# HighCWu/ControlLoRA

Hardware: AMD Instinct MI355X
Metric: train images/sec SD-1.5+ControlLoRA 512^2 bs4/GPU (higher is better)
Workload: dtype f16; 1 GPU; configs/fill50k.json on SD-1.5 topology (seeded random weights), 512x512, bs=4/GPU, fp16; hot path = hint encoder + UNet fwd/bwd + adapter AdamW; latents/text embeddings synthetic (VAE/CLIP outside the hot path); global_batch=4, parallelism=dp1, hipgraph=True, allreduce_bytes=24188160, rccl_ranks=1, comm=torch, comm_requested=auto

## Files before the change

controllora_amd/capi.py:

```python
from __future__ import annotations

import ctypes as C
import os
from typing import Optional

import torch

_HERE = os.path.dirname(os.path.abspath(__file__))
LIB_PATH = os.environ.get("CLORA_LIB_PATH") or os.path.join(_HERE, "_build", "libclora.so")

ABI_VERSION = 4
OK, ERR_ARG, ERR_LAUNCH, ERR_WORKSPACE = 0, -1, -2, -3
_ERR = {ERR_ARG: "bad argument", ERR_LAUNCH: "kernel launch failed", ERR_WORKSPACE: "workspace too small"}


class CloraError(RuntimeError):
    pass


class ConvDesc(C.Structure):
    _fields_ = [(n, C.c_int) for n in (
        "enabled", "Hin", "Win", "Cin", "Hout", "Wout", "ksize", "mul", "kmul", "off", "lim_h", "lim_w", "shift",
        "need_even", "kchunk")]

# ... 61 lines not shown

class LoraWgradJob(C.Structure):
    _fields_ = [("A", C.c_void_p), ("lda", C.c_int), ("T", C.c_void_p), ("ldt", C.c_int), ("toff", C.c_int), ("G", C.c_void_p),
                ("gs_n", C.c_int), ("gs_j", C.c_int), ("M", C.c_int), ("N", C.c_int), ("R", C.c_int), ("scale", C.c_float),
                ("a_rows", C.c_int), ("A2", C.c_void_p), ("lda2", C.c_int)]


class ConvPackJob(C.Structure):
    _fields_ = [("w", C.c_void_p), ("fwd", C.c_void_p), ("dgrad", C.c_void_p), ("Co", C.c_int), ("Ci", C.c_int), ("ksize", C.c_int),
                ("Cip", C.c_int), ("Cop", C.c_int), ("pad_", C.c_int)]


class ConvUnpackJob(C.Structure):
    _fields_ = [("stage", C.c_void_p), ("stage_b", C.c_void_p), ("grad_w", C.c_void_p), ("grad_b", C.c_void_p), ("Co", C.c_int),
                ("Ci", C.c_int), ("ksize", C.c_int), ("Cip", C.c_int)]


LORA_MAX_JOBS = 16
LORA_WGRAD_MAX_JOBS = 32
WGRAD_JOBS_PER_LAUNCH = min(LORA_WGRAD_MAX_JOBS, max(1, int(os.environ.get("CLORA_WGRAD_JOBS", "32"))))
CONV_MAX_JOBS = 32
CANNY_MAX_GROUP = 64
_P, _I, _Z, _F = C.c_void_p, C.c_int, C.c_size_t, C.c_float
_PROTOS = {
    "clora_gemm_f16": [_P, _I, _P, _P, _I, _I, _I, _I, C.POINTER(ConvDesc), C.POINTER(Epilogue), _I, _P, _Z, _P],
    "clora_gemm_f16_ex": [_P, _I, _P, _P, _I, _I, _I, _I, C.POINTER(ConvDesc), C.POINTER(Epilogue), _I, _I, _P, _Z, _P],
    "clora_conv_patch_eligible": [_I, C.POINTER(ConvDesc), _I],
    "clora_conv_strip_eligible": [_I, _I, C.POINTER(ConvDesc)],
    "clora_set_option": [C.c_char_p, _I],
    "clora_conv_wgrad_f16": [_P, _I, _P, _I, _P, _P, _I, _I, _I, C.POINTER(ConvDesc), _I, _P],
    "clora_conv_weight_pack_f32": [_P, _I, _I, _I, _I, _I, _P, _P, _P],
    "clora_conv_wgrad_unpack_f32": [_P, _P, _P, _P, _I, _I, _I, _I, _P],
    "clora_conv_weight_pack_multi_f32": [C.POINTER(ConvPackJob), _I, _P],
    "clora_conv_wgrad_unpack_multi_f32": [C.POINTER(ConvUnpackJob), _I, _P],
    "clora_attn_fwd_f16": [_P, _I, _P, _I, _P, _I, _P, _I, _P, _I, _I, _I, _I, _I, _F, _P],
    "clora_attn_max_head_dim": [_I],
    "clora_attn_fwd_causal_f16": [_P, _I, _P, _I, _P, _I, _P, _I, _I, _I, _I, _I, _F, _P],
    "clora_attn_bwd_f16": [_P, _I, _P, _I, _P, _I, _P, _I, _P, _I, _P, _P, _P, _I, _P, _I, _P, _I, _I, _I, _I, _I, _I, _F, _P, _Z, _P],
    "clora_groupnorm_fwd_f16": [_P, _P, _P, _P, _P, _I, _I, _I, _I, _F, _I, _P, _Z, _P],
    "clora_groupnorm_bwd_f16": [_P, _P, _P, _P, _P, _P, _P, _P, _P, _I, _I, _I, _I, _I, _I, _P, _Z, _P],
    "clora_groupnorm_fwd_f16_ex": [_P, _P, _I, C.POINTER(Deferred), _P, _P, _P, _P, _P, _I, _I, _I, _I, _F, _I, _P, _Z, _P],
    "clora_groupnorm_bwd_f16_ex": [_P, _P, C.POINTER(Deferred), _P, _P, _P, _I, _P, _P, _P, _P, _P, _I, _I, _I, _I, _I, _I, _P, _Z, _P],
    "clora_groupnorm_fwd_f16_team": [_P, _P, _I, C.POINTER(Deferred), _P, _P, _P, _P, _P, _I, _I, _I, _I, _F, _I, _P, _Z, _P, _Z, _P],
    "clora_groupnorm_fwd_f16_lo": [_P, _P, _I, C.POINTER(Deferred), _P, _P, _P, _P, _P, _I, _I, _I, _I, _F, _I, _P, _Z, _P, _Z, _P, _P, _P],
    "clora_layernorm_fwd_f16_lo": [_P, _P, _P, _P, _I, _I, _F, _P, _P],
    "clora_groupnorm_bwd_f16_team": [_P, _P, C.POINTER(Deferred), _P, _P, _P, _I, _P, _P, _P, _P, _P, _I, _I, _I, _I, _I, _I, _P, _Z, _P, _Z, _P],
    "clora_layernorm_bwd_f16_ex": [_P, _P, C.POINTER(Deferred), _P, _P, _P, _I, _I, _F, _P],
    "clora_finish_deferred": [C.POINTER(Deferred), _P],
    "clora_gemm_ln_fusable": [_I, _I, _I, _I, _I],
# ... 148 lines not shown
```

controllora_amd/csrc/clora_ew.hip:

```cpp
#include "clora_common.h"
#include "../../include/clora.h"

namespace {

int ew_grid(size_t work) {
    size_t b = (work + 255) / 256;
    return (int)(b > 4096 ? 4096 : (b < 1 ? 1 : b));
}

#define EW_LOOP(i, n) for (size_t i = (size_t)blockIdx.x * 256 + threadIdx.x; i < (n); i += (size_t)gridDim.x * 256)

__global__ __launch_bounds__(256) void add_kernel(const half_t* a, const half_t* b, half_t* y, size_t n8) {
    EW_LOOP(i, n8) {
        const half8 x = ld8(a + i * 8), z = ld8(b + i * 8);
        half8 o;
#pragma unroll
        for (int e = 0; e < 8; ++e) o[e] = (half_t)((float)x[e] + (float)z[e]);
        st8(y + i * 8, o);
    }
}

__global__ __launch_bounds__(256) void silu_kernel(const half_t* x, half_t* y, size_t n8) {
    EW_LOOP(i, n8) {
        const half8 v = ld8(x + i * 8);
// ... 384 lines not shown
#pragma unroll
    for (int q = 0; q < 8; ++q) s += acc[q][0] + acc[q][1] + acc[q][2] + acc[q][3];
    const unsigned long long c1 = CLORA_CYCLES(), w1 = CLORA_WALL_TICKS();
    if (threadIdx.x == 0) {
        out[3 * (size_t)blockIdx.x] = c1 - c0;
        out[3 * (size_t)blockIdx.x + 1] = w1 - w0;
        out[3 * (size_t)blockIdx.x + 2] = (unsigned long long)__float_as_uint(s);
    }
}
extern "C" int clora_clock_probe(unsigned long long* out, int blocks, int iters, void* stream) {
    if (!out || blocks <= 0 || iters <= 0) return CLORA_ERR_ARG;
    hipLaunchKernelGGL(clock_probe_kernel, dim3(blocks), dim3(256), 0, (hipStream_t)stream, out, iters);
    return clora_check_launch();
}
extern "C" int clora_abi_version(void) { return CLORA_ABI_VERSION; }
extern "C" const char* clora_build_info(void) { return "libclora gfx950 (v_mfma_f32_16x16x32_f16), ABI 2"; }

namespace {
struct ConvPackJobs { clora_conv_pack_job_t j[CLORA_CONV_MAX_JOBS]; };
struct ConvUnpackJobs { clora_conv_unpack_job_t j[CLORA_CONV_MAX_JOBS]; };

__global__ __launch_bounds__(256) void conv_weight_pack_multi_kernel(ConvPackJobs jobs) {
    const clora_conv_pack_job_t& p = jobs.j[blockIdx.y];
    const int taps = p.ksize * p.ksize, Co = p.Co, Ci = p.Ci, Cip = p.Cip, Cop = p.Cop;
    const float* w = p.w;
    half_t* fwd = (half_t*)p.fwd;
    half_t* dgrad = (half_t*)p.dgrad;
    const int nf = Co * taps * Cip, nd = dgrad ? Cip * taps * Cop : 0;
    for (int i = blockIdx.x * 256 + threadIdx.x; i < nf + nd; i += gridDim.x * 256) {
        if (i < nf) {
            const int ci = i % Cip, tap = (i / Cip) % taps, co = i / (Cip * taps);
// ... 11 lines not shown
    const int taps = p.ksize * p.ksize, Co = p.Co, Ci = p.Ci, Cip = p.Cip;
    const int nw = Co * taps * Cip;
    for (int i = blockIdx.x * 256 + threadIdx.x; i < nw + (p.grad_b ? Co : 0); i += gridDim.x * 256) {
        if (i < nw) {
            const int ci = i % Cip, tap = (i / Cip) % taps, co = i / (Cip * taps);
            const float v = p.stage[i];
            p.stage[i] = 0.f;
            if (ci < Ci) p.grad_w[((size_t)co * Ci + ci) * taps + tap] += v;
        } else {
            const int co = i - nw;
            p.grad_b[co] += p.stage_b[co];
            p.stage_b[co] = 0.f;
        }
    }
}
}

extern "C" int clora_conv_weight_pack_multi_f32(const clora_conv_pack_job_t* jobs, int njobs, void* stream) {
    if (!jobs || njobs <= 0 || njobs > CLORA_CONV_MAX_JOBS) return CLORA_ERR_ARG;
    ConvPackJobs cj;
    long most = 0;
    for (int i = 0; i < njobs; ++i) {
        const clora_conv_pack_job_t& j = jobs[i];
        if (!j.w || !j.fwd || j.Co <= 0 || j.Ci <= 0 || (j.ksize != 1 && j.ksize != 3) || j.Cip < j.Ci || (j.Cip & 7) ||
            (j.dgrad && (j.Cop < j.Co || (j.Cop & 7))))
            return CLORA_ERR_ARG;
        const int taps = j.ksize * j.ksize;
        const long total = (long)j.Co * taps * j.Cip + (j.dgrad ? (long)j.Cip * taps * j.Cop : 0);
        if (total > most) most = total;
        cj.j[i] = j;
// ... 26 lines not shown
```

controllora_amd/csrc/clora_gemm.hip:

```cpp
#include <string.h>
#include "clora_common.h"
#include "../../include/clora.h"
#include "clora_epilogue.h"

namespace {

struct GemmArgs {
    const half_t* A;
    const half_t* B;
    half_t* C;
    float* partial;
    int lda, ldc, M, N, K;
    int k_per_split;
    int tiles_n;
    int two_phase;
    int hoist_on;
    int tiles_m, n_major;
    int xg_s, xg_m, xg_n;
    clora_conv_t conv;
    clora_epilogue_t epi;
};

template <int BM, int BN, int WM, int WN>
__global__ __launch_bounds__(256) void gemm_kernel(GemmArgs p) {
// ... 1129 lines not shown
            st8(p.C + (size_t)m * p.ldc + n, finish_chunk8(p.partial, splits, p.M, p.N, p.epi, m, n));
        }
    }
}

struct WgradArgs {
    const half_t* dY;
    const half_t* X;
    float* dW;
    float* db;
    int ldy, ldx, M, N, K;
    int oihw_ci;
    int m_per_block;
    int tiles_n, tiles_k;
    clora_conv_t conv;
};

__device__ __attribute__((aligned(16))) const unsigned short g_clora_one16[8] = {0x3C00u, 0, 0, 0, 0, 0, 0, 0};

__global__ __launch_bounds__(256, 3) void conv_wgrad_kernel(WgradArgs p) {
    constexpr int BMR = 64, NST = 3;
    constexpr int SUB = BMR * 16;
    constexpr int STAGE = 8 * SUB;
    __shared__ __attribute__((aligned(16))) half_t smem[NST * STAGE];
    const int t = threadIdx.x;
    const int tile = blockIdx.x;
    const int tn = tile % p.tiles_n, tk = tile / p.tiles_n;
    const int n0 = tn * 64, k0 = tk * 64;
    const int mbeg = blockIdx.y * p.m_per_block;
    const int mend = (mbeg + p.m_per_block < p.M) ? mbeg + p.m_per_block : p.M;
    const int nst = (mend - mbeg + BMR - 1) / BMR;
    const bool conv = p.conv.enabled != 0;
    const half_t* zero_page = reinterpret_cast<const half_t*>(g_clora_zero16);
    const half_t* one_page = reinterpret_cast<const half_t*>(g_clora_one16);

    const int w = t >> 6, l = t & 63, g = l >> 4, li = l & 15;
    const int lm = (w & 1) * 32 + (l >> 1);
    const int c8 = (l & 1) * 8;
    int ncol[2], kcol[2], ky[2], kx[2], ci[2];
    bool n_ok[2], k_ok[2], k_one[2];
#pragma unroll
    for (int q = 0; q < 2; ++q) {
        const int sub = q * 2 + (w >> 1);
        ncol[q] = n0 + sub * 16 + c8;
        kcol[q] = k0 + sub * 16 + c8;
        n_ok[q] = ncol[q] < p.N;
        k_ok[q] = kcol[q] < p.K;
        k_one[q] = p.db != nullptr && kcol[q] == p.K;
        ky[q] = 0; kx[q] = 0; ci[q] = kcol[q];
        if (conv && k_ok[q]) {
            const int tap = kcol[q] / p.conv.Cin;
            ci[q] = kcol[q] - tap * p.conv.Cin;
            ky[q] = tap / p.conv.ksize;
            kx[q] = tap - ky[q] * p.conv.ksize;
        }
    }
    int mrow = mbeg + lm;
    auto issue_stage = [&](int buf) {
        half_t* base = smem + buf * STAGE + (w & 1) * 512;
        const bool mok = mrow < mend;
        size_t xrow = 0;
        int ty0 = 0, tx0 = 0;
        if (mok) {
// ... 71 lines not shown
#pragma unroll
            for (int i = 0; i < 2; ++i)
#pragma unroll
                for (int j = 0; j < 2; ++j) acc[i][j] = mfma16(af[i], bf[j], acc[i][j]);
        }
    }
    CLORA_WAIT_VMCNT(0);
#pragma unroll
    for (int i = 0; i < 2; ++i)
#pragma unroll
        for (int j = 0; j < 2; ++j)
#pragma unroll
            for (int r = 0; r < 4; ++r) {
                const int n = n0 + wm * 32 + i * 16 + 4 * g + r;
                const int kk = k0 + wn * 32 + j * 16 + li;
                if (n < p.N && kk < p.K) {
                    if (p.oihw_ci > 0) {
                        const int cin = p.conv.enabled ? p.conv.Cin : p.K;
                        const int tap = kk / cin, ci = kk - tap * cin;
                        const int taps = p.conv.enabled ? p.conv.ksize * p.conv.ksize : 1;
                        if (ci < p.oihw_ci) atomicAdd(p.dW + ((size_t)n * p.oihw_ci + ci) * taps + tap, acc[i][j][r]);
                    } else {
                        atomicAdd(p.dW + (size_t)n * p.K + kk, acc[i][j][r]);
                    }
                } else if (n < p.N && kk == p.K && p.db) atomicAdd(p.db + n, acc[i][j][r]);
            }
}

struct WgradPatchArgs {
    const half_t* dY;
    const half_t* X;
    float* dW;
    float* db;
    int N, K, H, W, nimg, nseg, rows_per_block, row_chunks;
    int Hin, Win;
};

template <int CIN, int NFW, int TW, int STRIDE = 1>
__global__ __launch_bounds__(CIN / 16 * 128) void conv_wgrad_patch_kernel(WgradPatchArgs p) {
    constexpr int WC = CIN / 16, NW = WC * 2, NP = 2 * NFW;
    constexpr int PW = STRIDE == 1 ? TW + 2 : 2 * TW + 1, PPIX = 3 * PW;
    constexpr int P_NI = (PPIX * 2 + 63) / 64;
    constexpr int PLANE = P_NI * 512;
    constexpr int Y_NI = TW * 2 / 64, YPLANE = TW * 16;
    constexpr int BUF = WC * PLANE + NP * YPLANE;
    constexpr int NI = WC * P_NI + NP * Y_NI, NIW = (NI + NW - 1) / NW;
    constexpr int KS = TW / 32;
    static_assert((2 * BUF + 512) * 2 <= 160 * 1024, "LDS per workgroup");
    __shared__ __attribute__((aligned(16))) half_t smem[2 * BUF + 512];
    const int t = threadIdx.x, w = t >> 6, l = t & 63, g = l >> 4, li = l & 15;
    const int cb = w >> 1, wn = w & 1;
    const half_t* zero_page = reinterpret_cast<const half_t*>(g_clora_zero16);

// ... 88 lines not shown
                const half_t* q = P + (ky * PW + koff + s * 32) * 16 + troff;
                const half4v lo = CLORA_DS_READ_TR16(q), hi = CLORA_DS_READ_TR16(q + 64);
                const half8 bf = half8{lo[0], lo[1], lo[2], lo[3], hi[0], hi[1], hi[2], hi[3]};
#pragma unroll
                for (int f = 0; f < NFW; ++f) acc[tap][f] = mfma16(af[f], bf, acc[tap][f]);
            }
        }
        CLORA_RAW_BARRIER();
    }
    CLORA_WAIT_VMCNT(0);
#pragma unroll
    for (int f = 0; f < NFW; ++f)
#pragma unroll
        for (int r = 0; r < 4; ++r) {
            const int n = (wn * NFW + f) * 16 + 4 * g + r;
            if (n < p.N) {
#pragma unroll
                for (int tap = 0; tap < 9; ++tap) atomicAdd(p.dW + (size_t)n * p.K + tap * CIN + cb * 16 + li, acc[tap][f][r]);
                if (cb == 0 && li == 0 && p.db) atomicAdd(p.db + n, accb[f][r]);
            }
        }
}

template <int CIN, int NFW, int TW, int STRIDE = 1>
int launch_wgrad_patch(WgradPatchArgs& a, hipStream_t s) {
    a.nseg = a.W / TW;
    const long strips = (long)a.nimg * a.nseg;
    long target = 4700000L / ((long)a.N * (a.K + 1));
    target = target < 64 ? 64 : (target > 512 ? 512 : target);
    if (clora_option(CLORA_OPT_WGRAD_PATCH) >= 64) target = clora_option(CLORA_OPT_WGRAD_PATCH);
    long rpb = ((long)a.H * strips + target - 1) / target;
    if (rpb < 4) rpb = 4;
    if (rpb > a.H) rpb = a.H;
    a.rows_per_block = (int)rpb;
    a.row_chunks = clora_cdiv(a.H, rpb);
    hipLaunchKernelGGL((conv_wgrad_patch_kernel<CIN, NFW, TW, STRIDE>), dim3((unsigned)(strips * a.row_chunks)), dim3(CIN / 16 * 128), 0, s, a);
    return clora_check_launch();
}

struct StripArgs {
    const half_t* X;
    const half_t* Wt;
    half_t* C;
    const float* bias;
    int N, ldc, H, W, nimg, nseg, rows_per_block, row_chunks;
    int off, kmul;
};

template <int CIN, int NF, int TW>
__global__ __launch_bounds__(256) void conv3x3_strip_kernel(StripArgs p) {
    constexpr int WC = CIN / 16, NW = 4, KSTEPS = CIN / 32;
// ... 774 lines not shown
}

extern "C" int clora_conv_weight_pack_f32(const float* w, int Co, int Ci, int ksize, int Cip, int Cop, clora_half* fwd,
                                          clora_half* dgrad, void* stream) {
    if (!w || !fwd || Co <= 0 || Ci <= 0 || (ksize != 1 && ksize != 3) || Cip < Ci || (Cip & 7) || (dgrad && (Cop < Co || (Cop & 7))))
        return CLORA_ERR_ARG;
    const int taps = ksize * ksize;
    const long total = (long)Co * taps * Cip + (dgrad ? (long)Cip * taps * Cop : 0);
    int blocks = (int)((total + 255) / 256);
    if (blocks > 2048) blocks = 2048;
    hipLaunchKernelGGL(conv_weight_pack_kernel, dim3(blocks), dim3(256), 0, (hipStream_t)stream, w, Co, Ci, taps, Cip, Cop,
                       (half_t*)fwd, (half_t*)dgrad);
    return clora_check_launch();
}

extern "C" int clora_conv_wgrad_f16(const clora_half* dY, int ldy, const clora_half* X, int ldx, float* dW, float* db,
                                    int M, int N, int K, const clora_conv_t* conv, int oihw_ci, void* stream) {
    if (!dY || !X || !dW || M <= 0 || N <= 0 || K <= 0 || (K & 7) || (N & 7) || (ldy & 7) || oihw_ci < 0) return CLORA_ERR_ARG;
    WgradArgs a;
    a.dY = (const half_t*)dY; a.X = (const half_t*)X; a.dW = dW; a.db = db;
    a.ldy = ldy; a.ldx = ldx; a.M = M; a.N = N; a.K = K; a.oihw_ci = oihw_ci;
    if (conv && conv->enabled) {
        a.conv = *conv;
        if ((conv->Cin & 7) || K != conv->ksize * conv->ksize * conv->Cin || conv->kchunk != 0) return CLORA_ERR_ARG;
    } else {
        a.conv = clora_conv_t();
        a.conv.enabled = 0;
        if (ldx & 7) return CLORA_ERR_ARG;
    }
    if (conv && conv->enabled && clora_option(CLORA_OPT_WGRAD_PATCH) && oihw_ci == 0 && ldy == N) {
        const clora_conv_t& c = *conv;
        const bool s1 = c.ksize == 3 && c.mul == 1 && c.kmul == 1 && c.off == -1 && c.shift == 0 && c.need_even == 0 && c.Hout == c.Hin &&
                        c.Wout == c.Win && c.lim_h == c.Hin && c.lim_w == c.Win && c.Hout > 0 && (M % (c.Hout * c.Wout)) == 0 &&
                        (long)M * (c.Cin > N ? c.Cin : N) < (1L << 31);
        const bool s2 = c.ksize == 3 && c.mul == 2 && c.kmul == 1 && c.off == 0 && c.shift == 0 && c.need_even == 0 && c.Hin == 2 * c.Hout &&
                        c.Win == 2 * c.Wout && c.lim_h == c.Hin && c.lim_w == c.Win && c.Hout > 0 && (M % (c.Hout * c.Wout)) == 0 &&
                        (long)M * 4 * (c.Cin > N ? c.Cin : N) < (1L << 31);
        if ((s1 || s2) && (c.Cin == 32 || c.Cin == 64) && N <= 64) {
            WgradPatchArgs q;
            q.dY = (const half_t*)dY; q.X = (const half_t*)X; q.dW = dW; q.db = db; q.N = N; q.K = K; q.H = c.Hout; q.W = c.Wout;
            q.Hin = c.Hin; q.Win = c.Win;
            q.nimg = M / (c.Hout * c.Wout);
            hipStream_t s = (hipStream_t)stream;
            if (s2) {
                if (c.Cin == 32 && N <= 32 && (c.Wout % 64) == 0) return launch_wgrad_patch<32, 1, 64, 2>(q, s);
                if (c.Cin == 32 && N <= 64 && (c.Wout % 64) == 0) return launch_wgrad_patch<32, 2, 64, 2>(q, s);
                if (c.Cin == 64 && N <= 64 && (c.Wout % 64) == 0) return launch_wgrad_patch<64, 2, 64, 2>(q, s);
            } else {
            if (c.Cin == 32 && N <= 32 && (c.Wout % 128) == 0) return launch_wgrad_patch<32, 1, 128>(q, s);
            if (c.Cin == 32 && N <= 64 && (c.Wout % 128) == 0) return launch_wgrad_patch<32, 2, 128>(q, s);
            if (c.Cin == 32 && N <= 64 && (c.Wout % 64) == 0) return launch_wgrad_patch<32, 2, 64>(q, s);
            if (c.Cin == 64 && N <= 64 && (c.Wout % 64) == 0) return launch_wgrad_patch<64, 2, 64>(q, s);
            }
        }
    }
    a.tiles_n = clora_cdiv(N, 64);
    a.tiles_k = clora_cdiv(K + (db ? 8 : 0), 64);
    const int tiles = a.tiles_n * a.tiles_k;
    int chunks = clora_cdiv(2048, tiles);
    int mpb = clora_cdiv(clora_cdiv(M, chunks), 64) * 64;
    if (mpb < 256) mpb = 256;
    a.m_per_block = mpb;
    hipLaunchKernelGGL(conv_wgrad_kernel, dim3(tiles, clora_cdiv(M, mpb)), dim3(256), 0, (hipStream_t)stream, a);
    return clora_check_launch();
}
```

controllora_amd/kernels.py:

```python
from __future__ import annotations

import ctypes as C
import os
from typing import Optional, Tuple

import torch

from . import capi
from .capi import ConvDesc, Epilogue, ptr

f16, f32 = torch.float16, torch.float32


class KernelProfiler:

    def __init__(self, detail=False):
        self.detail = detail
        self.records = []

    def summary(self):
        torch.cuda.synchronize()
        agg = {}
        for name, e0, e1, fl, by in self.records:
            a = agg.setdefault(name, dict(calls=0, ms=0.0, flops=0.0, bytes=0.0))
# ... 328 lines not shown

def conv_wgrad_staged(dY, X, M, N, K, conv, stage: torch.Tensor, weight_grad: torch.Tensor, bias_grad: Optional[torch.Tensor], Cip: int):
    assert stage.dtype == f32 and stage.numel() == N * K + N and weight_grad.dtype == f32 and weight_grad.is_contiguous()
    sw, sb = stage[:N * K], stage[N * K:]
    _call("clora_conv_wgrad_f16", ptr(dY, f16), N, ptr(X, f16), K, ptr(sw), ptr(sb), M, N, K,
          C.byref(conv) if conv is not None else None, 0, flops=2.0 * M * N * K)
    if bias_grad is not None and conv_unpack_defer(conv_unpack_job(stage, weight_grad, bias_grad, Cip), stage, weight_grad, bias_grad):
        return
    Co, Ci, k, _ = weight_grad.shape
    _call("clora_conv_wgrad_unpack_f32", ptr(sw), ptr(sb) if bias_grad is not None else None, ptr(weight_grad),
          ptr(bias_grad, f32) if bias_grad is not None else None, Co, Ci, k, Cip)
    if bias_grad is None:
        sb.zero_()


def conv_weight_pack(weight: torch.Tensor, Cip: int, need_dgrad: bool, out=None):
    Co, Ci, k, _ = weight.shape
    Cop = (Co + 7) // 8 * 8
    if out is not None:
        fwd, dgrad = out
    else:
        fwd = torch.empty((Co, k * k * Cip), dtype=f16, device=weight.device)
        dgrad = torch.empty((Cip, k * k * Cop), dtype=f16, device=weight.device) if need_dgrad else None
    _call("clora_conv_weight_pack_f32", ptr(weight, f32), Co, Ci, k, Cip, Cop, ptr(fwd), ptr(dgrad) if dgrad is not None else None)
    return fwd, dgrad


def conv_pack_job(weight: torch.Tensor, Cip: int, fwd: torch.Tensor, dgrad: Optional[torch.Tensor]):
    Co, Ci, k, _ = weight.shape
    assert weight.dtype == f32 and weight.is_contiguous() and fwd.dtype == f16 and fwd.numel() == Co * k * k * Cip
# ... 301 lines not shown


def lora_wgrad_multi(jobs, device):
    groups = {}
    for j in jobs:
        groups.setdefault(4 if j.R <= 4 else (8 if j.R <= 8 else 16), []).append(j)
    wsb = capi.lib().cdll.clora_lora_wgrad_workspace_bytes
    for _, js in groups.items():
        for i in range(0, len(js), capi.WGRAD_JOBS_PER_LAUNCH):
            chunk = js[i:i + capi.WGRAD_JOBS_PER_LAUNCH]
            ws = workspace(sum(wsb(j.M, j.N, j.R) for j in chunk), device)
            arr = (capi.LoraWgradJob * len(chunk))(*chunk)
            _call("clora_lora_wgrad_multi_f16", arr, len(chunk), ptr(ws), ws.numel(), nbytes=sum(2.0 * j.M * j.N for j in chunk))


_wgrad_queue = {"jobs": [], "refs": [], "task": None, "enabled": os.environ.get("CLORA_DEFER_WGRAD", "1") != "0", "unpack": []}
DEFER_UNPACK = os.environ.get("CLORA_DEFER_UNPACK", "1") != "0"


def _graph_task_id():
    f = getattr(torch._C, "_current_graph_task_id", None)
    return f() if f is not None else -1


def _defer_open():
    if not _wgrad_queue["enabled"] or PROFILER is not None:
        return False
    task = _graph_task_id()
    if task < 0:
        return False
    if _wgrad_queue["task"] != task:
# ... 8 lines not shown
        lora_wgrad_multi(jobs, device)
        return
    _wgrad_queue["jobs"].extend(jobs)
    _wgrad_queue["refs"].extend(keepalive)
    _wgrad_queue["device"] = device


def conv_unpack_defer(job, *keepalive) -> bool:
    if not DEFER_UNPACK or not _defer_open():
        return False
    _wgrad_queue["unpack"].append(job)
    _wgrad_queue["refs"].extend(keepalive)
    return True


def lora_wgrad_discard():
    _wgrad_queue["jobs"].clear()
    _wgrad_queue["unpack"].clear()
    _wgrad_queue["refs"].clear()
    _wgrad_queue["task"] = None


def lora_wgrad_flush():
    jobs, _wgrad_queue["jobs"] = _wgrad_queue["jobs"], []
    unpack, _wgrad_queue["unpack"] = _wgrad_queue["unpack"], []
    _wgrad_queue["task"] = None
    if unpack:
        conv_wgrad_unpack_multi(unpack)
    if jobs:
        batches = []
        for j in jobs:
            for b in batches:
                if len(b[0]) < capi.WGRAD_JOBS_PER_LAUNCH and j.G not in b[1] and b[2] == (4 if j.R <= 4 else (8 if j.R <= 8 else 16)):
                    b[0].append(j); b[1].add(j.G)
                    break
            else:
                batches.append(([j], {j.G}, 4 if j.R <= 4 else (8 if j.R <= 8 else 16)))
        for b in batches:
            lora_wgrad_multi(b[0], _wgrad_queue["device"])
    _wgrad_queue["refs"].clear()


def lora_up(base, T, toff, U, M, N, scale, out=None, u_tr=False):
# ... 187 lines not shown
```

controllora_amd/ops.py:

```python
from __future__ import annotations

from typing import List, Optional, Sequence, Tuple

import torch

from . import kernels as K

f16, f32 = torch.float16, torch.float32


class LinearPack:

    def __init__(self, weight: torch.Tensor, bias: Optional[torch.Tensor], pad_n_to: int = 8):
        w = weight.detach().reshape(weight.shape[0], -1).to(f16)
        N, Kd = w.shape
        if Kd % 8:
            w = torch.cat([w, w.new_zeros(N, 8 - Kd % 8)], 1)
            Kd = w.shape[1]
        Np = (N + pad_n_to - 1) // pad_n_to * pad_n_to
        if Np != N:
            w = torch.cat([w, w.new_zeros(Np - N, Kd)], 0)
        self.N, self.K, self.N_logical = Np, Kd, N
        self.w = w.contiguous()
        self.wt = w.t().contiguous()
# ... 1305 lines not shown
                K.lora_wgrad(a_, t_, 0, g_, gn, gj, M, n_, R, scale=sc_)
        dbase, dx = dy, None
        if ctx.same:
            if ctx.needs_input_grad[0] or ctx.needs_input_grad[1]:
                dbase = K.lora_up(dy, dT, 0, D.detach(), M, D.shape[1], 1.0, u_tr=True)
            return dbase, None, None, None, None
        if ctx.needs_input_grad[1]:
            dx = K.lora_up(None, dT, 0, D.detach(), M, D.shape[1], 1.0, u_tr=True)
        return dbase, dx, None, None, None


def lora_apply(base, x, down_weight, up_weight, scale):
    return _LoraApplyFn.apply(base, x, down_weight, up_weight, float(scale))


class _TrainConvFn(torch.autograd.Function):

    @staticmethod
    def forward(ctx, x, weight, bias, B, H, W, stride, asym_pad, need_dx):
        Co, Ci, k, _ = weight.shape
        Cip = x.shape[1]
        if PERSISTENT_CONV_PACKS:
            wp, wd = TRAIN_CONV_PACKS.get(weight, Cip, need_dx)
        else:
            wp, wd = K.conv_weight_pack(weight.detach(), Cip, need_dx)
        if k == 3:
            cd, Ho, Wo = K.conv_fwd_desc(H, W, Cip, 3, stride, 0 if asym_pad else 1, False, asym_pad)
            y = K.gemm(x, wp, B * Ho * Wo, Co, 9 * Cip, conv=cd, bias=bias.detach())
        else:
            cd, Ho, Wo = None, H, W
# ... 10 lines not shown
        weight, bias = ctx.params
        B, H, W, Ho, Wo, stride, asym_pad, need_dx, cd = ctx.cfg
        Co, Ci, k, _ = weight.shape
        Cip = x.shape[1]
        Cop = (Co + 7) // 8 * 8
        M = B * Ho * Wo
        dx = None
        if need_dx:
            if k == 3:
                cdd = K.conv_dgrad_desc(Ho, Wo, Cop, H, W, 3, stride, 1, asym_pad)
                dx = K.gemm(dy, ctx.wd, B * H * W, Cip, 9 * Cop, conv=cdd)
            else:
                dx = K.gemm(dy, ctx.wd, M, Cip, Cop)
        if weight.requires_grad:
            gb = _grad_buffer(bias) if bias.requires_grad else None
            if k == 1:
                K.conv_wgrad_into(dy, x, M, Co, Cip, cd, _grad_buffer(weight), gb)
            else:
                stage = getattr(weight, "_clora_wgrad_stage", None)
                if stage is None or stage.numel() != Co * 9 * Cip + Co or stage.device != dy.device:
                    stage = torch.zeros(Co * 9 * Cip + Co, dtype=f32, device=dy.device)
                    weight._clora_wgrad_stage = stage
                K.conv_wgrad_staged(dy, x, M, Co, 9 * Cip, cd, stage, _grad_buffer(weight), gb, Cip)
        return dx, None, None, None, None, None, None, None, None


def train_conv(x, weight, bias, B, H, W, stride=1, asym_pad=False, need_dx=True):
    return _TrainConvFn.apply(x, weight, bias, B, H, W, stride, asym_pad, need_dx)
```

include/clora.h:

```cpp
#ifndef CLORA_H
#define CLORA_H
#include <stddef.h>
#include <stdint.h>

#ifdef __cplusplus
extern "C" {
#endif

#define CLORA_OK 0
#define CLORA_ERR_ARG (-1)
#define CLORA_ERR_LAUNCH (-2)
#define CLORA_ERR_WORKSPACE (-3)

typedef uint16_t clora_half;

typedef struct {
    int enabled;
    int Hin, Win, Cin;
    int Hout, Wout;
    int ksize;
    int mul, kmul, off, lim_h, lim_w, shift, need_even;
    int kchunk;
} clora_conv_t;

// ... 97 lines not shown
    const float* w;
    clora_half* fwd;
    clora_half* dgrad;
    int Co, Ci, ksize, Cip, Cop, pad_;
} clora_conv_pack_job_t;
int clora_conv_weight_pack_multi_f32(const clora_conv_pack_job_t* jobs, int njobs, void* stream);
typedef struct {
    float* stage;
    float* stage_b;
    float* grad_w;
    float* grad_b;
    int Co, Ci, ksize, Cip;
} clora_conv_unpack_job_t;
int clora_conv_wgrad_unpack_multi_f32(const clora_conv_unpack_job_t* jobs, int njobs, void* stream);

int clora_attn_fwd_f16(const clora_half* q, int ldq, const clora_half* k, int ldk, const clora_half* v, int ldv,
                       clora_half* o, int ldo, float* lse, int B, int H, int Nq, int Nk, int D, float scale,
                       void* stream);
int clora_attn_max_head_dim(int backward);
int clora_attn_fwd_causal_f16(const clora_half* q, int ldq, const clora_half* k, int ldk, const clora_half* v, int ldv,
                              clora_half* o, int ldo, int B, int H, int N, int D, float scale, void* stream);
int clora_attn_bwd_f16(const clora_half* q, int ldq, const clora_half* k, int ldk, const clora_half* v, int ldv,
                       const clora_half* o, int ldo, const clora_half* dO, int lddo, const float* lse,
                       float* delta, clora_half* dq, int lddq, clora_half* dk, int lddk, clora_half* dv, int lddv,
                       int B, int H, int Nq, int Nk, int D, float scale, void* workspace, size_t workspace_bytes,
                       void* stream);

int clora_groupnorm_fwd_f16(const clora_half* x, clora_half* y, const float* gamma, const float* beta, float* stats,
                            int B, int HW, int C, int G, float eps, int fuse_silu, void* workspace,
                            size_t workspace_bytes, void* stream);
// ... 154 lines not shown
```

Before: 184.2 images/s.

## Replace atomic conv weight-grad accumulation with per-chunk slabs and deferred fold

Conv weight-gradient kernels now write partial sums into per-row-chunk fp32 slabs in a workspace instead of atomically adding into the gradient, or staging then unpacking. A new multi-job fold kernel reduces the slabs, converts them to OIHW layout and accumulates into grad_w/grad_b, and it can be deferred and batched with the other wgrad flush work. The aim is to remove atomic contention and the separate stage/unpack pass. In exchange it adds workspace memory and an extra read of every slab. It is enabled by default through CLORA_WGRAD_SLABS.

```diff
diff --git a/controllora_amd/capi.py b/controllora_amd/capi.py
--- a/controllora_amd/capi.py
+++ b/controllora_amd/capi.py
@@ -99,6 +99,17 @@
 class ConvUnpackJob(C.Structure):
     _fields_ = [("stage", C.c_void_p), ("stage_b", C.c_void_p), ("grad_w", C.c_void_p), ("grad_b", C.c_void_p), ("Co", C.c_int),
                 ("Ci", C.c_int), ("ksize", C.c_int), ("Cip", C.c_int)]
+
+
+class WgradPlan(C.Structure):
+    _fields_ = [("kernel", C.c_int), ("blocks", C.c_int), ("row_chunks", C.c_int), ("rows_per_chunk", C.c_int), ("nslabs", C.c_int),
+                ("kw", C.c_int), ("slab_stride", C.c_int), ("patch_cin", C.c_int), ("patch_nfw", C.c_int), ("patch_tw", C.c_int),
+                ("patch_stride", C.c_int), ("workspace_bytes", C.c_size_t)]
+
+
+class ConvFoldJob(C.Structure):
+    _fields_ = [("slabs", C.c_void_p), ("grad_w", C.c_void_p), ("grad_b", C.c_void_p), ("nslabs", C.c_int), ("kw", C.c_int),
+                ("slab_stride", C.c_int), ("Co", C.c_int), ("Ci", C.c_int), ("ksize", C.c_int), ("Cip", C.c_int)]
 
 
 LORA_MAX_JOBS = 16
@@ -118,6 +129,9 @@
     "clora_conv_wgrad_unpack_f32": [_P, _P, _P, _P, _I, _I, _I, _I, _P],
     "clora_conv_weight_pack_multi_f32": [C.POINTER(ConvPackJob), _I, _P],
     "clora_conv_wgrad_unpack_multi_f32": [C.POINTER(ConvUnpackJob), _I, _P],
+    "clora_conv_wgrad_slab_plan": [_I, _I, _I, C.POINTER(ConvDesc), _I, _I, C.POINTER(WgradPlan)],
+    "clora_conv_wgrad_slabs_f16": [_P, _P, _I, _I, _I, C.POINTER(ConvDesc), _I, _I, _P, _Z, _P],
+    "clora_conv_wgrad_fold_multi_f32": [C.POINTER(ConvFoldJob), _I, _P],
     "clora_attn_fwd_f16": [_P, _I, _P, _I, _P, _I, _P, _I, _P, _I, _I, _I, _I, _I, _F, _P],
     "clora_attn_max_head_dim": [_I],
     "clora_attn_fwd_causal_f16": [_P, _I, _P, _I, _P, _I, _P, _I, _I, _I, _I, _I, _F, _P],
diff --git a/controllora_amd/csrc/clora_ew.hip b/controllora_amd/csrc/clora_ew.hip
--- a/controllora_amd/csrc/clora_ew.hip
+++ b/controllora_amd/csrc/clora_ew.hip
@@ -422,7 +422,9 @@
     return clora_check_launch();
 }
 extern "C" int clora_abi_version(void) { return CLORA_ABI_VERSION; }
-extern "C" const char* clora_build_info(void) { return "libclora gfx950 (v_mfma_f32_16x16x32_f16), ABI 2"; }
+#define CLORA_STR_(x) #x
+#define CLORA_STR(x) CLORA_STR_(x)
+extern "C" const char* clora_build_info(void) { return "libclora gfx950 (v_mfma_f32_16x16x32_f16), ABI " CLORA_STR(CLORA_ABI_VERSION); }
 
 namespace {
 struct ConvPackJobs { clora_conv_pack_job_t j[CLORA_CONV_MAX_JOBS]; };
@@ -464,6 +466,80 @@
         }
     }
 }
+struct ConvFoldJobs { clora_conv_fold_job_t j[CLORA_CONV_MAX_JOBS]; int lanes[CLORA_CONV_MAX_JOBS]; };
+
+__global__ __launch_bounds__(256) void conv_wgrad_fold_multi_kernel(ConvFoldJobs jobs) {
+    __shared__ floatx4 red[256];
+    const clora_conv_fold_job_t& p = jobs.j[blockIdx.y];
+    const int L = jobs.lanes[blockIdx.y], EPB = 256 / L;
+    const int t = threadIdx.x, e = t % EPB, q = t / EPB;
+    const int taps = p.ksize * p.ksize, kq = taps * p.Cip / 4;
+    const int nq = p.Co * kq, total = nq + (p.grad_b ? p.Co : 0);
+    const size_t stride = (size_t)p.slab_stride;
+    for (int base = blockIdx.x * EPB; base < total; base += gridDim.x * EPB) {
+        const int i = base + e;
+        int co = 0, col = 0;
+        floatx4 s = zero4f();
+        if (i < nq) {
+            co = i / kq; col = (i - co * kq) * 4;
+            const float* src = p.slabs + (size_t)co * p.kw + col;
+            for (int b = q; b < p.nslabs; b += 8 * L) {
+                floatx4 v[8];
+#pragma unroll
+                for (int u = 0; u < 8; ++u)
+                    v[u] = (b + u * L < p.nslabs) ? *reinterpret_cast<const floatx4*>(src + (size_t)(b + u * L) * stride) : zero4f();
+#pragma unroll
+                for (int u = 0; u < 8; ++u) s += v[u];
+            }
+        } else if (i < total) {
+            co = i - nq;
+            const float* src = p.slabs + (size_t)co * p.kw + kq * 4;
+            for (int b = q; b < p.nslabs; b += L) s[0] += src[(size_t)b * stride];
+        }
+        red[t] = s;
+        __syncthreads();
+        if (q == 0 && i < total) {
+            for (int u = 1; u < L; ++u) {
+                s += red[u * EPB + e];
+            }
+            if (i < nq) {
+                const int tap = col / p.Cip, ci = col - tap * p.Cip;
+                float* dst = p.grad_w + ((size_t)co * p.Ci + ci) * taps + tap;
+                if (ci < p.Ci) dst[0] += s[0];
+                if (ci + 1 < p.Ci) dst[taps] += s[1];
+                if (ci + 2 < p.Ci) dst[2 * taps] += s[2];
+                if (ci + 3 < p.Ci) dst[3 * taps] += s[3];
+            } else {
+                p.grad_b[co] += s[0];
+            }
+        }
+        __syncthreads();
+    }
+}
+}
+
+extern "C" int clora_conv_wgrad_fold_multi_f32(const clora_conv_fold_job_t* jobs, int njobs, void* stream) {
+    if (!jobs || njobs <= 0 || njobs > CLORA_CONV_MAX_JOBS) return CLORA_ERR_ARG;
+    ConvFoldJobs cj;
+    int most = 0;
+    for (int i = 0; i < njobs; ++i) {
+        const clora_conv_fold_job_t& j = jobs[i];
+        if (!j.slabs || !j.grad_w || j.Co <= 0 || j.Ci <= 0 || j.Cip < j.Ci || (j.ksize != 1 && j.ksize != 3) || j.nslabs <= 0) return CLORA_ERR_ARG;
+        const long kcols = (long)j.ksize * j.ksize * j.Cip;
+        if (j.kw != kcols + (j.grad_b ? 8 : 0) || (long)j.slab_stride != (long)j.Co * j.kw) return CLORA_ERR_ARG;
+        for (int k = 0; k < i; ++k)
+            if (jobs[k].grad_w == j.grad_w) return CLORA_ERR_ARG;
+        if ((j.Cip & 3) || ((size_t)j.slabs & 15)) return CLORA_ERR_ARG;
+        int L = 1;
+        while (L < 32 && j.nslabs > 8 * L) L *= 2;
+        const int groups = clora_cdiv((long)j.Co * kcols / 4 + (j.grad_b ? j.Co : 0), 256 / L);
+        if (groups > most) most = groups;
+        cj.j[i] = j;
+        cj.lanes[i] = L;
+    }
+    if (most > 2048) most = 2048;
+    hipLaunchKernelGGL(conv_wgrad_fold_multi_kernel, dim3(most, njobs), dim3(256), 0, (hipStream_t)stream, cj);
+    return clora_check_launch();
 }
 
 extern "C" int clora_conv_weight_pack_multi_f32(const clora_conv_pack_job_t* jobs, int njobs, void* stream) {
diff --git a/controllora_amd/csrc/clora_gemm.hip b/controllora_amd/csrc/clora_gemm.hip
--- a/controllora_amd/csrc/clora_gemm.hip
+++ b/controllora_amd/csrc/clora_gemm.hip
@@ -1167,10 +1167,13 @@
     int m_per_block;
     int tiles_n, tiles_k;
     clora_conv_t conv;
+    int has_bias;
+    int kw, slab_stride;
 };
 
 __device__ __attribute__((aligned(16))) const unsigned short g_clora_one16[8] = {0x3C00u, 0, 0, 0, 0, 0, 0, 0};
 
+template <bool SLAB>
 __global__ __launch_bounds__(256, 3) void conv_wgrad_kernel(WgradArgs p) {
     constexpr int BMR = 64, NST = 3;
     constexpr int SUB = BMR * 16;
@@ -1199,7 +1202,7 @@
         kcol[q] = k0 + sub * 16 + c8;
         n_ok[q] = ncol[q] < p.N;
         k_ok[q] = kcol[q] < p.K;
-        k_one[q] = p.db != nullptr && kcol[q] == p.K;
+        k_one[q] = p.has_bias && kcol[q] == p.K;
         ky[q] = 0; kx[q] = 0; ci[q] = kcol[q];
         if (conv && k_ok[q]) {
             const int tap = kcol[q] / p.conv.Cin;
@@ -1301,7 +1304,10 @@
             for (int r = 0; r < 4; ++r) {
                 const int n = n0 + wm * 32 + i * 16 + 4 * g + r;
                 const int kk = k0 + wn * 32 + j * 16 + li;
-                if (n < p.N && kk < p.K) {
+                if constexpr (SLAB) {
+                    if (n < p.N && (kk < p.K || (kk == p.K && p.has_bias)))
+                        p.dW[(size_t)blockIdx.y * p.slab_stride + (size_t)n * p.kw + kk] = acc[i][j][r];
+                } else if (n < p.N && kk < p.K) {
                     if (p.oihw_ci > 0) {
                         const int cin = p.conv.enabled ? p.conv.Cin : p.K;
                         const int tap = kk / cin, ci = kk - tap * cin;
@@ -1321,9 +1327,10 @@
     float* db;
     int N, K, H, W, nimg, nseg, rows_per_block, row_chunks;
     int Hin, Win;
+    int has_bias, kw, slab_stride;
 };
 
-template <int CIN, int NFW, int TW, int STRIDE = 1>
+template <int CIN, int NFW, int TW, int STRIDE = 1, bool SLAB = false>
 __global__ __launch_bounds__(CIN / 16 * 128) void conv_wgrad_patch_kernel(WgradPatchArgs p) {
     constexpr int WC = CIN / 16, NW = WC * 2, NP = 2 * NFW;
     constexpr int PW = STRIDE == 1 ? TW + 2 : 2 * TW + 1, PPIX = 3 * PW;
@@ -1442,7 +1449,14 @@
 #pragma unroll
         for (int r = 0; r < 4; ++r) {
             const int n = (wn * NFW + f) * 16 + 4 * g + r;
-            if (n < p.N) {
+            if constexpr (SLAB) {
+                if (n < p.N) {
+                    float* row = p.dW + (size_t)blockIdx.x * p.slab_stride + (size_t)n * p.kw;
+#pragma unroll
+                    for (int tap = 0; tap < 9; ++tap) row[tap * CIN + cb * 16 + li] = acc[tap][f][r];
+                    if (cb == 0 && li == 0 && p.has_bias) row[p.K] = accb[f][r];
+                }
+            } else if (n < p.N) {
 #pragma unroll
                 for (int tap = 0; tap < 9; ++tap) atomicAdd(p.dW + (size_t)n * p.K + tap * CIN + cb * 16 + li, acc[tap][f][r]);
                 if (cb == 0 && li == 0 && p.db) atomicAdd(p.db + n, accb[f][r]);
@@ -1450,19 +1464,28 @@
         }
 }
 
-template <int CIN, int NFW, int TW, int STRIDE = 1>
+constexpr int WGRAD_SLAB_PATCH_BLOCKS = 512;
+constexpr int WGRAD_SLAB_GATHER_BLOCKS = 2048, WGRAD_SLAB_GATHER_MIN_ROWS = 512, WGRAD_SLAB_GATHER_MAX_CHUNKS = 256;
+static void wgrad_patch_blocks(int N, int K, int H, long strips, bool slab, int chunks, int* rows_per_block, int* row_chunks) {
+    long target = slab ? WGRAD_SLAB_PATCH_BLOCKS : 4700000L / ((long)N * (K + 1));
+    if (!slab) target = target < 64 ? 64 : (target > 512 ? 512 : target);
+    const bool forced = clora_option(CLORA_OPT_WGRAD_PATCH) >= 64;
+    if (forced) target = clora_option(CLORA_OPT_WGRAD_PATCH);
+    long rpb = ((long)H * strips + target - 1) / target;
+    const long least = (slab && !forced) ? 8 : 4;
+    if (rpb < least) rpb = least;
+    if (slab && chunks > 0) rpb = clora_cdiv(H, chunks);
+    if (rpb > H) rpb = H;
+    *rows_per_block = (int)rpb;
+    *row_chunks = clora_cdiv(H, (int)rpb);
+}
+
+template <int CIN, int NFW, int TW, int STRIDE = 1, bool SLAB = false>
 int launch_wgrad_patch(WgradPatchArgs& a, hipStream_t s) {
     a.nseg = a.W / TW;
     const long strips = (long)a.nimg * a.nseg;
-    long target = 4700000L / ((long)a.N * (a.K + 1));
-    target = target < 64 ? 64 : (target > 512 ? 512 : target);
-    if (clora_option(CLORA_OPT_WGRAD_PATCH) >= 64) target = clora_option(CLORA_OPT_WGRAD_PATCH);
-    long rpb = ((long)a.H * strips + target - 1) / target;
-    if (rpb < 4) rpb = 4;
-    if (rpb > a.H) rpb = a.H;
-    a.rows_per_block = (int)rpb;
-    a.row_chunks = clora_cdiv(a.H, rpb);
-    hipLaunchKernelGGL((conv_wgrad_patch_kernel<CIN, NFW, TW, STRIDE>), dim3((unsigned)(strips * a.row_chunks)), dim3(CIN / 16 * 128), 0, s, a);
+    if (!SLAB) wgrad_patch_blocks(a.N, a.K, a.H, strips, false, 0, &a.rows_per_block, &a.row_chunks);
+    hipLaunchKernelGGL((conv_wgrad_patch_kernel<CIN, NFW, TW, STRIDE, SLAB>), dim3((unsigned)(strips * a.row_chunks)), dim3(CIN / 16 * 128), 0, s, a);
     return clora_check_launch();
 }
 
@@ -2267,6 +2290,42 @@
     return clora_check_launch();
 }
 
+struct WgradPatchPick { int cin, nfw, tw, stride; };
+static bool wgrad_patch_pick(int M, int N, const clora_conv_t* conv, bool wide, WgradPatchPick* k) {
+    if (!conv || !conv->enabled || !clora_option(CLORA_OPT_WGRAD_PATCH)) return false;
+    const clora_conv_t& c = *conv;
+    const bool s1 = c.ksize == 3 && c.mul == 1 && c.kmul == 1 && c.off == -1 && c.shift == 0 && c.need_even == 0 && c.Hout == c.Hin &&
+                    c.Wout == c.Win && c.lim_h == c.Hin && c.lim_w == c.Win && c.Hout > 0 && (M % (c.Hout * c.Wout)) == 0 &&
+                    (long)M * (c.Cin > N ? c.Cin : N) < (1L << 31);
+    const bool s2 = c.ksize == 3 && c.mul == 2 && c.kmul == 1 && c.off == 0 && c.shift == 0 && c.need_even == 0 && c.Hin == 2 * c.Hout &&
+                    c.Win == 2 * c.Wout && c.lim_h == c.Hin && c.lim_w == c.Win && c.Hout > 0 && (M % (c.Hout * c.Wout)) == 0 &&
+                    (long)M * 4 * (c.Cin > N ? c.Cin : N) < (1L << 31);
+    if (!(s1 || s2) || (c.Cin != 32 && c.Cin != 64)) return false;
+    const int nfw = N <= 32 ? 1 : (N <= 64 ? 2 : 4);
+    if (s2) {
+        if (N > 64 || (c.Wout % 64)) return false;
+        *k = WgradPatchPick{c.Cin, c.Cin == 64 ? 2 : nfw, 64, 2};
+        return true;
+    }
+    if (c.Cin == 32 && N <= 64 && (c.Wout % 128) == 0) { *k = WgradPatchPick{32, nfw, 128, 1}; return true; }
+    if (c.Cin == 32 && N <= 64 && (c.Wout % 64) == 0) { *k = WgradPatchPick{32, 2, 64, 1}; return true; }
+    if (c.Cin == 64 && N <= 64 && (c.Wout % 64) == 0) { *k = WgradPatchPick{64, 2, 64, 1}; return true; }
+    if (wide && c.Cin == 64 && N <= 128 && (c.Wout % 64) == 0) { *k = WgradPatchPick{64, 4, 64, 1}; return true; }
+    return false;
+}
+
+template <bool SLAB>
+static int launch_wgrad_patch_pick(const WgradPatchPick& k, WgradPatchArgs& q, hipStream_t s) {
+#define CLORA_WGRAD_PATCH_CASE(CIN, NFW, TW, ST) \
+    if (k.cin == CIN && k.nfw == NFW && k.tw == TW && k.stride == ST) return launch_wgrad_patch<CIN, NFW, TW, ST, SLAB>(q, s);
+    CLORA_WGRAD_PATCH_CASE(32, 1, 64, 2) CLORA_WGRAD_PATCH_CASE(32, 2, 64, 2) CLORA_WGRAD_PATCH_CASE(64, 2, 64, 2)
+    CLORA_WGRAD_PATCH_CASE(32, 1, 128, 1) CLORA_WGRAD_PATCH_CASE(32, 2, 128, 1) CLORA_WGRAD_PATCH_CASE(32, 2, 64, 1)
+    CLORA_WGRAD_PATCH_CASE(64, 2, 64, 1)
+    if constexpr (SLAB) { CLORA_WGRAD_PATCH_CASE(64, 4, 64, 1) }
+#undef CLORA_WGRAD_PATCH_CASE
+    return CLORA_ERR_ARG;
+}
+
 extern "C" int clora_conv_wgrad_f16(const clora_half* dY, int ldy, const clora_half* X, int ldx, float* dW, float* db,
                                     int M, int N, int K, const clora_conv_t* conv, int oihw_ci, void* stream) {
     if (!dY || !X || !dW || M <= 0 || N <= 0 || K <= 0 || (K & 7) || (N & 7) || (ldy & 7) || oihw_ci < 0) return CLORA_ERR_ARG;
@@ -2281,31 +2340,16 @@
         a.conv.enabled = 0;
         if (ldx & 7) return CLORA_ERR_ARG;
     }
-    if (conv && conv->enabled && clora_option(CLORA_OPT_WGRAD_PATCH) && oihw_ci == 0 && ldy == N) {
+    a.has_bias = db != nullptr; a.kw = 0; a.slab_stride = 0;
+    WgradPatchPick pick;
+    if (oihw_ci == 0 && ldy == N && wgrad_patch_pick(M, N, conv, false, &pick)) {
         const clora_conv_t& c = *conv;
-        const bool s1 = c.ksize == 3 && c.mul == 1 && c.kmul == 1 && c.off == -1 && c.shift == 0 && c.need_even == 0 && c.Hout == c.Hin &&
-                        c.Wout == c.Win && c.lim_h == c.Hin && c.lim_w == c.Win && c.Hout > 0 && (M % (c.Hout * c.Wout)) == 0 &&
-                        (long)M * (c.Cin > N ? c.Cin : N) < (1L << 31);
-        const bool s2 = c.ksize == 3 && c.mul == 2 && c.kmul == 1 && c.off == 0 && c.shift == 0 && c.need_even == 0 && c.Hin == 2 * c.Hout &&
-                        c.Win == 2 * c.Wout && c.lim_h == c.Hin && c.lim_w == c.Win && c.Hout > 0 && (M % (c.Hout * c.Wout)) == 0 &&
-                        (long)M * 4 * (c.Cin > N ? c.Cin : N) < (1L << 31);
-        if ((s1 || s2) && (c.Cin == 32 || c.Cin == 64) && N <= 64) {
-            WgradPatchArgs q;
-            q.dY = (const half_t*)dY; q.X = (const half_t*)X; q.dW = dW; q.db = db; q.N = N; q.K = K; q.H = c.Hout; q.W = c.Wout;
-            q.Hin = c.Hin; q.Win = c.Win;
-            q.nimg = M / (c.Hout * c.Wout);
-            hipStream_t s = (hipStream_t)stream;
-            if (s2) {
-                if (c.Cin == 32 && N <= 32 && (c.Wout % 64) == 0) return launch_wgrad_patch<32, 1, 64, 2>(q, s);
-                if (c.Cin == 32 && N <= 64 && (c.Wout % 64) == 0) return launch_wgrad_patch<32, 2, 64, 2>(q, s);
-                if (c.Cin == 64 && N <= 64 && (c.Wout % 64) == 0) return launch_wgrad_patch<64, 2, 64, 2>(q, s);
-            } else {
-            if (c.Cin == 32 && N <= 32 && (c.Wout % 128) == 0) return launch_wgrad_patch<32, 1, 128>(q, s);
-            if (c.Cin == 32 && N <= 64 && (c.Wout % 128) == 0) return launch_wgrad_patch<32, 2, 128>(q, s);
-            if (c.Cin == 32 && N <= 64 && (c.Wout % 64) == 0) return launch_wgrad_patch<32, 2, 64>(q, s);
-            if (c.Cin == 64 && N <= 64 && (c.Wout % 64) == 0) return launch_wgrad_patch<64, 2, 64>(q, s);
-            }
-        }
+        WgradPatchArgs q;
+        q.dY = (const half_t*)dY; q.X = (const half_t*)X; q.dW = dW; q.db = db; q.N = N; q.K = K; q.H = c.Hout; q.W = c.Wout;
+        q.Hin = c.Hin; q.Win = c.Win;
+        q.nimg = M / (c.Hout * c.Wout);
+        q.has_bias = db != nullptr; q.kw = 0; q.slab_stride = 0;
+        return launch_wgrad_patch_pick<false>(pick, q, (hipStream_t)stream);
     }
     a.tiles_n = clora_cdiv(N, 64);
     a.tiles_k = clora_cdiv(K + (db ? 8 : 0), 64);
@@ -2314,6 +2358,72 @@
     int mpb = clora_cdiv(clora_cdiv(M, chunks), 64) * 64;
     if (mpb < 256) mpb = 256;
     a.m_per_block = mpb;
-    hipLaunchKernelGGL(conv_wgrad_kernel, dim3(tiles, clora_cdiv(M, mpb)), dim3(256), 0, (hipStream_t)stream, a);
+    hipLaunchKernelGGL(conv_wgrad_kernel<false>, dim3(tiles, clora_cdiv(M, mpb)), dim3(256), 0, (hipStream_t)stream, a);
     return clora_check_launch();
 }
+
+static int wgrad_conv_args_ok(int M, int N, int K, const clora_conv_t* conv) {
+    if (M <= 0 || N <= 0 || K <= 0 || (K & 7) || (N & 7)) return 0;
+    if (conv && conv->enabled && ((conv->Cin & 7) || K != conv->ksize * conv->ksize * conv->Cin || conv->kchunk != 0)) return 0;
+    return 1;
+}
+
+extern "C" int clora_conv_wgrad_slab_plan(int M, int N, int K, const clora_conv_t* conv, int with_bias, int chunks, clora_wgrad_plan_t* plan) {
+    if (!plan || chunks < 0 || !wgrad_conv_args_ok(M, N, K, conv)) return CLORA_ERR_ARG;
+    clora_wgrad_plan_t& p = *plan;
+    p = clora_wgrad_plan_t();
+    p.kw = K + (with_bias ? 8 : 0);
+    if ((long)N * p.kw >= (1L << 31)) return CLORA_ERR_ARG;
+    p.slab_stride = N * p.kw;
+    WgradPatchPick pick;
+    if (wgrad_patch_pick(M, N, conv, true, &pick)) {
+        const long strips = (long)(M / (conv->Hout * conv->Wout)) * (conv->Wout / pick.tw);
+        p.kernel = 1;
+        p.patch_cin = pick.cin; p.patch_nfw = pick.nfw; p.patch_tw = pick.tw; p.patch_stride = pick.stride;
+        wgrad_patch_blocks(N, K, conv->Hout, strips, true, chunks, &p.rows_per_chunk, &p.row_chunks);
+        p.blocks = (int)(strips * p.row_chunks);
+        p.nslabs = p.blocks;
+    } else {
+        const int tiles = clora_cdiv(N, 64) * clora_cdiv(p.kw, 64);
+        int want = chunks > 0 ? chunks : clora_cdiv(WGRAD_SLAB_GATHER_BLOCKS, tiles);
+        if (chunks == 0 && want > WGRAD_SLAB_GATHER_MAX_CHUNKS) want = WGRAD_SLAB_GATHER_MAX_CHUNKS;
+        int mpb = clora_cdiv(clora_cdiv(M, want), 64) * 64;
+        if (mpb < WGRAD_SLAB_GATHER_MIN_ROWS && chunks == 0) mpb = WGRAD_SLAB_GATHER_MIN_ROWS;
+        p.kernel = 0;
+        p.rows_per_chunk = mpb;
+        p.row_chunks = clora_cdiv(M, mpb);
+        p.blocks = tiles * p.row_chunks;
+        p.nslabs = p.row_chunks;
+    }
+    p.workspace_bytes = (size_t)p.nslabs * p.slab_stride * sizeof(float);
+    return CLORA_OK;
+}
+
+extern "C" int clora_conv_wgrad_slabs_f16(const clora_half* dY, const clora_half* X, int M, int N, int K, const clora_conv_t* conv,
+                                          int with_bias, int chunks, float* workspace, size_t workspace_bytes, void* stream) {
+    clora_wgrad_plan_t p;
+    if (!dY || !X || !workspace) return CLORA_ERR_ARG;
+    if (int rc = clora_conv_wgrad_slab_plan(M, N, K, conv, with_bias, chunks, &p)) return rc;
+    if (workspace_bytes < p.workspace_bytes) return CLORA_ERR_WORKSPACE;
+    if (p.kernel == 1) {
+        const clora_conv_t& c = *conv;
+        WgradPatchArgs q;
+        q.dY = (const half_t*)dY; q.X = (const half_t*)X; q.dW = workspace; q.db = nullptr; q.N = N; q.K = K; q.H = c.Hout; q.W = c.Wout;
+        q.Hin = c.Hin; q.Win = c.Win;
+        q.nimg = M / (c.Hout * c.Wout);
+        q.has_bias = with_bias != 0; q.kw = p.kw; q.slab_stride = p.slab_stride;
+        q.rows_per_block = p.rows_per_chunk; q.row_chunks = p.row_chunks;
+        return launch_wgrad_patch_pick<true>(WgradPatchPick{p.patch_cin, p.patch_nfw, p.patch_tw, p.patch_stride}, q, (hipStream_t)stream);
+    }
+    WgradArgs a;
+    a.dY = (const half_t*)dY; a.X = (const half_t*)X; a.dW = workspace; a.db = nullptr;
+    a.ldy = N; a.ldx = K; a.M = M; a.N = N; a.K = K; a.oihw_ci = 0;
+    if (conv && conv->enabled) a.conv = *conv;
+    else { a.conv = clora_conv_t(); a.conv.enabled = 0; }
+    a.has_bias = with_bias != 0; a.kw = p.kw; a.slab_stride = p.slab_stride;
+    a.tiles_n = clora_cdiv(N, 64);
+    a.tiles_k = clora_cdiv(p.kw, 64);
+    a.m_per_block = p.rows_per_chunk;
+    hipLaunchKernelGGL(conv_wgrad_kernel<true>, dim3(a.tiles_n * a.tiles_k, p.row_chunks), dim3(256), 0, (hipStream_t)stream, a);
+    return clora_check_launch();
+}
diff --git a/controllora_amd/kernels.py b/controllora_amd/kernels.py
--- a/controllora_amd/kernels.py
+++ b/controllora_amd/kernels.py
@@ -366,6 +366,50 @@
         sb.zero_()
 
 
+WGRAD_SLABS = os.environ.get("CLORA_WGRAD_SLABS", "1") != "0"
+
+
+def conv_wgrad_plan(M: int, N: int, K: int, conv: Optional[ConvDesc], with_bias: bool, chunks: int = 0) -> capi.WgradPlan:
+    plan = capi.WgradPlan()
+    capi.lib().call("clora_conv_wgrad_slab_plan", M, N, K, C.byref(conv) if conv is not None else None, int(with_bias), int(chunks),
+                    C.byref(plan))
+    return plan
+
+
+def conv_fold_job(ws: torch.Tensor, plan: capi.WgradPlan, weight_grad: torch.Tensor, bias_grad: Optional[torch.Tensor], Cip: int):
+    Co, Ci, k, _ = weight_grad.shape
+    assert weight_grad.dtype == f32 and weight_grad.is_contiguous() and ws.dtype == f32 and ws.numel() * 4 >= plan.workspace_bytes
+    assert plan.kw == k * k * Cip + (8 if bias_grad is not None else 0) and plan.slab_stride == Co * plan.kw
+    return capi.ConvFoldJob(ptr(ws), ptr(weight_grad), ptr(bias_grad, f32) if bias_grad is not None else None, plan.nslabs, plan.kw,
+                            plan.slab_stride, Co, Ci, k, Cip)
+
+
+def conv_wgrad_fold_multi(jobs):
+    for i in range(0, len(jobs), capi.CONV_MAX_JOBS):
+        chunk = jobs[i:i + capi.CONV_MAX_JOBS]
+        arr = (capi.ConvFoldJob * len(chunk))(*chunk)
+        _call("clora_conv_wgrad_fold_multi_f32", arr, len(chunk), nbytes=sum(4.0 * j.nslabs * j.slab_stride for j in chunk))
+
+
+def conv_wgrad_slabs_launch(dY, X, M, N, K, conv, with_bias: bool, ws: torch.Tensor, chunks: int = 0):
+    assert ws.dtype == f32 and dY.dtype == f16 and X.dtype == f16 and dY.is_contiguous() and X.is_contiguous()
+    _call("clora_conv_wgrad_slabs_f16", ptr(dY, f16), ptr(X, f16), M, N, K, C.byref(conv) if conv is not None else None,
+          int(with_bias), int(chunks), ptr(ws), ws.numel() * 4, flops=2.0 * M * N * K)
+
+
+def conv_wgrad_slabs(dY, X, M, N, K, conv, ws: torch.Tensor, weight_grad: torch.Tensor, bias_grad: Optional[torch.Tensor], Cip: int,
+                     chunks: int = 0):
+    plan = conv_wgrad_plan(M, N, K, conv, bias_grad is not None, chunks)
+    job = conv_fold_job(ws, plan, weight_grad, bias_grad, Cip)
+    deferred = conv_fold_open(job)
+    conv_wgrad_slabs_launch(dY, X, M, N, K, conv, bias_grad is not None, ws, chunks)
+    if deferred:
+        conv_fold_defer(job, ws, weight_grad, bias_grad)
+    else:
+        conv_wgrad_fold_multi([job])
+    return plan
+
+
 def conv_weight_pack(weight: torch.Tensor, Cip: int, need_dgrad: bool, out=None):
     Co, Ci, k, _ = weight.shape
     Cop = (Co + 7) // 8 * 8
@@ -697,7 +741,7 @@
             _call("clora_lora_wgrad_multi_f16", arr, len(chunk), ptr(ws), ws.numel(), nbytes=sum(2.0 * j.M * j.N for j in chunk))
 
 
-_wgrad_queue = {"jobs": [], "refs": [], "task": None, "enabled": os.environ.get("CLORA_DEFER_WGRAD", "1") != "0", "unpack": []}
+_wgrad_queue = {"jobs": [], "refs": [], "task": None, "enabled": os.environ.get("CLORA_DEFER_WGRAD", "1") != "0", "unpack": [], "fold": []}
 DEFER_UNPACK = os.environ.get("CLORA_DEFER_UNPACK", "1") != "0"
 
 
@@ -736,9 +780,27 @@
     return True
 
 
+def conv_fold_open(job) -> bool:
+    if not DEFER_UNPACK or not _defer_open():
+        return False
+    q = _wgrad_queue["fold"]
+    clash = [j for j in q if j.slabs == job.slabs or j.grad_w == job.grad_w]
+    if clash:
+        q[:] = [j for j in q if not (j.slabs == job.slabs or j.grad_w == job.grad_w)]
+        for j in clash:
+            conv_wgrad_fold_multi([j])
+    return True
+
+
+def conv_fold_defer(job, *keepalive):
+    _wgrad_queue["fold"].append(job)
+    _wgrad_queue["refs"].extend(keepalive)
+
+
 def lora_wgrad_discard():
     _wgrad_queue["jobs"].clear()
     _wgrad_queue["unpack"].clear()
+    _wgrad_queue["fold"].clear()
     _wgrad_queue["refs"].clear()
     _wgrad_queue["task"] = None
 
@@ -746,9 +808,12 @@
 def lora_wgrad_flush():
     jobs, _wgrad_queue["jobs"] = _wgrad_queue["jobs"], []
     unpack, _wgrad_queue["unpack"] = _wgrad_queue["unpack"], []
+    fold, _wgrad_queue["fold"] = _wgrad_queue["fold"], []
     _wgrad_queue["task"] = None
     if unpack:
         conv_wgrad_unpack_multi(unpack)
+    if fold:
+        conv_wgrad_fold_multi(fold)
     if jobs:
         batches = []
         for j in jobs:
diff --git a/controllora_amd/ops.py b/controllora_amd/ops.py
--- a/controllora_amd/ops.py
+++ b/controllora_amd/ops.py
@@ -1343,6 +1343,19 @@
     return _LoraApplyFn.apply(base, x, down_weight, up_weight, float(scale))
 
 
+_WGRAD_WS_RETIRED = []
+
+
+def _wgrad_slab_workspace(weight, nbytes, device):
+    ws = getattr(weight, "_clora_wgrad_ws", None)
+    if ws is None or ws.numel() * 4 < nbytes or ws.device != device:
+        if ws is not None:
+            _WGRAD_WS_RETIRED.append(ws)
+        ws = torch.empty((nbytes + 3) // 4, dtype=f32, device=device)
+        weight._clora_wgrad_ws = ws
+    return ws
+
+
 class _TrainConvFn(torch.autograd.Function):
 
     @staticmethod
@@ -1383,7 +1396,11 @@
                 dx = K.gemm(dy, ctx.wd, M, Cip, Cop)
         if weight.requires_grad:
             gb = _grad_buffer(bias) if bias.requires_grad else None
-            if k == 1:
+            if K.WGRAD_SLABS:
+                plan = K.conv_wgrad_plan(M, Co, k * k * Cip, cd, gb is not None)
+                K.conv_wgrad_slabs(dy, x, M, Co, k * k * Cip, cd, _wgrad_slab_workspace(weight, plan.workspace_bytes, dy.device),
+                                   _grad_buffer(weight), gb, Cip)
+            elif k == 1:
                 K.conv_wgrad_into(dy, x, M, Co, Cip, cd, _grad_buffer(weight), gb)
             else:
                 stage = getattr(weight, "_clora_wgrad_stage", None)
diff --git a/include/clora.h b/include/clora.h
--- a/include/clora.h
+++ b/include/clora.h
@@ -135,6 +135,29 @@
 } clora_conv_unpack_job_t;
 int clora_conv_wgrad_unpack_multi_f32(const clora_conv_unpack_job_t* jobs, int njobs, void* stream);
 
+typedef struct {
+    int kernel;
+    int blocks;
+    int row_chunks;
+    int rows_per_chunk;
+    int nslabs;
+    int kw;
+    int slab_stride;
+    int patch_cin, patch_nfw, patch_tw, patch_stride;
+    size_t workspace_bytes;
+} clora_wgrad_plan_t;
+int clora_conv_wgrad_slab_plan(int M, int N, int K, const clora_conv_t* conv, int with_bias, int chunks, clora_wgrad_plan_t* plan);
+int clora_conv_wgrad_slabs_f16(const clora_half* dY, const clora_half* X, int M, int N, int K, const clora_conv_t* conv,
+                               int with_bias, int chunks, float* workspace, size_t workspace_bytes, void* stream);
+typedef struct {
+    const float* slabs;
+    float* grad_w;
+    float* grad_b;
+    int nslabs, kw, slab_stride;
+    int Co, Ci, ksize, Cip;
+} clora_conv_fold_job_t;
+int clora_conv_wgrad_fold_multi_f32(const clora_conv_fold_job_t* jobs, int njobs, void* stream);
+
 int clora_attn_fwd_f16(const clora_half* q, int ldq, const clora_half* k, int ldk, const clora_half* v, int ldv,
                        clora_half* o, int ldo, float* lse, int B, int H, int Nq, int Nk, int D, float scale,
                        void* stream);
```

Measured after the change: 185.5 images/s (median of 6 runs). About the same (+0.7%).
